# linhthi/BLISS-GNN

Measured on AMD Instinct MI355X. Metric: steps/sec (train step: sample_blocks + gather + SAGE fwd/bwd + Adam + exp3), reddit-like, higher is better.
Workload: dtype bf16

## Files before the change

bliss_gnn_amd/_lib.py:

```python
import ctypes as C
import os

_HERE = os.path.dirname(os.path.abspath(__file__))
LIB_PATH = os.path.join(_HERE, "libbliss_gnn.so")

EINVAL = -1
MODE_BANDIT, MODE_LADIES, MODE_UNIFORM_NODES, MODE_PARTIALS = 0, 1, 4, 8

ERR_BITS = {
    1: "frontier larger than 2^31-1 edges",
    2: "candidate capacity exceeded / seed id out of range",
    4: "kept-node capacity exceeded",
    8: "block-edge capacity exceeded",
    16: "non-finite or negative weight reached an exact reduction",
    32: "exact sum left its fixed-point range",
    64: "seed capacity exceeded",
    128: "random stream ran short / generator made no progress",
    256: "a cross-stream flag never came (bliss_flag_wait timed out)",
}


class Graph(C.Structure):
    _fields_ = [("indptr", C.c_void_p), ("indices", C.c_void_p), ("eid", C.c_void_p),
                ("num_nodes", C.c_int32), ("num_edges", C.c_int64)]
# ... 67 lines not shown
                ("rows_bound", C.c_int32), ("rows_dev", C.c_void_p),
                ("dw", C.c_void_p), ("dw_stride", C.c_int64), ("db", C.c_void_p)]


class GatFused(C.Structure):
    _fields_ = [("indptr", C.c_void_p), ("src", C.c_void_p), ("n_dst", C.c_int32), ("n_dst_dev", C.c_void_p),
                ("feat", C.c_void_p), ("feat_stride", C.c_int64), ("attn", C.c_void_p), ("heads", C.c_int32), ("head_dim", C.c_int32),
                ("negative_slope", C.c_float), ("e", C.c_void_p), ("a", C.c_void_p), ("a_drop", C.c_void_p),
                ("rst", C.c_void_p), ("rst_stride", C.c_int64),
                ("drop_p", C.c_float), ("drop_seed", C.c_uint32), ("drop_ctr", C.c_void_p), ("drop_ctr_used", C.c_void_p),
                ("g", C.c_void_p), ("g_stride", C.c_int64), ("de", C.c_void_p), ("d_er", C.c_void_p), ("d_er_stride", C.c_int64),
                ("dattn_part", C.c_void_p),
                ("wg_row", C.c_void_p), ("n_wg_dev", C.c_void_p), ("cap_wg", C.c_int32), ("row_ws", C.c_void_p), ("seg_part", C.c_void_p),
                ("err", C.c_void_p)]


ADAM_MAX_TENSORS = 32


class AdamTensors(C.Structure):
    _fields_ = [("param", C.c_void_p * ADAM_MAX_TENSORS), ("grad", C.c_void_p * ADAM_MAX_TENSORS),
                ("exp_avg", C.c_void_p * ADAM_MAX_TENSORS), ("exp_avg_sq", C.c_void_p * ADAM_MAX_TENSORS),
                ("numel", C.c_int64 * ADAM_MAX_TENSORS), ("count", C.c_int32)]


class BlockOut(C.Structure):
    _fields_ = [("indptr", C.c_void_p), ("src", C.c_void_p), ("dst", C.c_void_p), ("pos", C.c_void_p),
                ("eid", C.c_void_p), ("edge_weights", C.c_void_p), ("q_ij", C.c_void_p), ("t_indptr", C.c_void_p),
                ("t_edge", C.c_void_p), ("t_scratch", C.c_void_p), ("cap_b", C.c_int32)]


_P, _I32, _I64, _F, _D = C.c_void_p, C.c_int32, C.c_int64, C.c_float, C.c_double

SIGNATURES = {
    "bliss_layer_counts_bytes": [],
    "bliss_frontier_prob": [C.POINTER(Graph), C.POINTER(NodeMaps), _P, _P, _I32, _P, _I32, C.c_int, _F, _F, _I64, C.POINTER(LayerWs), _P],
    "bliss_rng_stream_begin": [_P, _P, _P, _P, _I32, _P],
    "bliss_rng_stream_wait": [_P, _P, _P, C.c_int, _I32, _P],
    "bliss_rng_stream_end": [_P, _P, _P, _I32, _P, _P],
    "bliss_rng_stream_chain": [_P, _P, _P, _P, _I32, _P, _I32, _P, _P],
    "bliss_rng_stream_ready": [_P],
    "bliss_rng_prepare": [_I32, _P],
    "bliss_mt_jump_poly": [_I64, _P],
    "bliss_flag_wait": [_P, _P, _P],
    "bliss_flag_set_spin_bound": [C.c_int64],
    "bliss_flag_raise": [_P, _P],
    "bliss_gather_rows": [_P, _I64, _P, _I32, _I32, _P, _I64, _P, _P],
    "bliss_exp3_apply_ranks": [C.POINTER(Exp3RankLists), _P, _P, _P, _P],
    "bliss_pack_lists": [C.POINTER(PackLists), _P, _P],
    "bliss_mt19937_uniform": [_P, _P, _I32, _P, _I32, _P],
    "bliss_poisson_select": [C.POINTER(LayerWs), _I32, _D, _P, _P, _P, C.c_int, _I32, _I64, _P],
    "bliss_multinomial_select": [C.POINTER(LayerWs), _P, _I32, _P],
    "bliss_tile_gemm": [C.POINTER(TileGemm), C.POINTER(TileGemm), _P],
    "bliss_cross_entropy": [_P, _I64, _P, _I32, _I32, _P, _P, _I64, _P, _P, _P, _P],
    "bliss_cross_entropy_sum": [_P, _I64, _P, _I64, _P, _P, _I32, _I32, _P, _P, _I64, _P, _P, _P, _P],
    "bliss_cross_entropy_masked": [_P, _I64, _P, _I64, _P, _I32, _P, _I32, _I32, _P, _F, _I32, _P, _P, _I64, _P, _P, _P, _P],
    "bliss_adam_step": [C.POINTER(AdamTensors), _P, _F, _F, _F, _F, _P],
    "bliss_cand_importance": [_P, _I32, C.c_int, _P, _P, _P],
    "bliss_poisson_scale": [_P, _P, _I32, _D, _P, _P],
    "bliss_keyed_select": [_P, _P, _P, _I32, _P, C.c_uint64, C.c_uint64, _I32, _P, _P, _P],
    "bliss_exp3_normalize_global": [_P, _I64, _P, _P, _P, _P, _P],
    "bliss_build_block": [C.POINTER(Graph), C.POINTER(NodeMaps), _P, _P, _I32, C.c_int, _F, _F, _I64, C.POINTER(LayerWs), C.POINTER(BlockOut), _P],
    "bliss_normalized_edata": [C.POINTER(Graph), _P, _P],
    "bliss_embed_norm": [_P, _I32, _I32, _I64, _P, _P],
    "bliss_spmm_fwd": [_P, _P, _P, _P, _P, _I64, _I32, _P, _I32, _I32, C.c_int, _P, _I64, C.c_int, _P, _P],
    "bliss_spmm_bwd": [_P, _P, _P, _P, _P, _P, _P, _I64, _I32, _P, _I32, _I32, C.c_int, _P, _I64, C.c_int, _P, _P],
    "bliss_block_transpose": [_P, _P, _I32, _I32, _I32, _P, _P, _P, _I64, _P],
    "bliss_spmm_chunk_edges": [_I32],
    "bliss_sage_epilogue_fwd": [_P, _I64, _P, _I64, _I32, _I32, _F, C.c_uint32, _P, _P, _I64, _P, _P],
    "bliss_sage_epilogue_bwd": [_P, _I64, _P, _I64, _I32, _I32, _F, _P, _I64, _P],
    "bliss_gat_chunk_edges": [],
    "bliss_graph_prepare": [_P, _P, _I64, _I32, C.c_int, _P, _P, _P, _P, _P, _P, _I64, _P],
    "bliss_exp3_update": [C.POINTER(Graph), _P, _P, _P, _P, _P, _P, _P, _P, _P, _P, _P, _P, _I32, _P, _I32, _F, _P, _P, C.c_int, _P, _P],
    "bliss_exp3_step": [C.POINTER(Graph), _P, C.POINTER(Exp3Block), _I32, _F, _P, _P],
    "bliss_exp3_normalize_global_rows": [C.POINTER(Exp3Block), _I32, _I64, _P, _I64, _P],
    "bliss_exp3_update_blocks": [C.POINTER(Graph), _P, C.POINTER(Exp3Block), _I32, _F, _P, _P],
    "bliss_exp3_apply": [_P, _P, _P, _P, _P, _I32, _P, _P],
    "bliss_exp3_normalize": [_P, _I64, _P, _P, _P, _P],
    "bliss_row_sum": [_P, _I64, _P, _P],
    "bliss_gat_logits": [_P, _P, _P, _I32, _P, _I64, _P, _I32, _I32, _F, _P, _P],
    "bliss_sage_dgrad": [C.POINTER(DGrad), _P],
    "bliss_sage_wgrad": [C.POINTER(WGrad), _I32, _P, _I64, _P],
    "bliss_shard_local_seeds": [_P, _I32, _P, _I32, _I32, _I32, _P, _P, _P, _P, _P, _P],
    "bliss_shard_scatter_partials": [_P, _P, _P, _P, _P, _P, _P, _I32, _P, _P],
    "bliss_shard_zero_dense": [_P, _I32, _P],
    "bliss_shard_pack_rows": [_P, _P, _I32, _I32, _I32, _P, _I64, _I32, _P, _I64, _P],
    "bliss_shard_place_rows": [_P, _I64, _P, _P, _I32, _P, _I64, _I32, _I32, _P],
    "bliss_shard_take_rows": [_P, _I32, _I64, _I32, _P, _P, _I32, _P, _I64, _I32, _P],
    "bliss_shard_candidates": [_P, _I32, _I32, _P, _P, _P, _P, _P, _I32, _P, _P, _P],
    "bliss_shard_select_kept": [_P, _P, _P, _P, C.c_uint64, _P, _I32, _P, _I32, _P, _P, _P, _P, _P, _I32, _I32, _I32, _P, _P, _P, _I32, _P, _P, _P],
    "bliss_gat_fused_supported": [_I32, _I32],
    "bliss_gat_segment_edges": [],
    "bliss_gat_fused_stamps": [_P, _P],
    "bliss_gat_segments": [_P, _I32, _I32, _P, _P, _P, _P],
    "bliss_gat_fused_fwd": [C.POINTER(GatFused), _P],
    "bliss_gat_fused_bwd_dst": [C.POINTER(GatFused), _P, _P, _P, _P],
    "bliss_gat_rows_src_fused": [_P, _I32, _P, _P, _P, _P, _I32, _P, _P, _P, _I64, _P, _I64, _P, _I32, _I32, _F, _P, _I64, _P, _P],
    "bliss_gat_logits_f32": [_P, _P, _P, _I32, _P, _I64, _P, _I32, _I32, _F, _P, _P],
    "bliss_gat_edge_dot": [_P, _P, _P, _I32, _P, _I64, _P, _I64, _I32, _I32, _P, _P],
    "bliss_gat_edge_softmax": [_P, _I32, _P, _P, _I32, C.c_int, _P, _P],
    "bliss_gat_rows": [C.c_int, _P, _I32, _P, _P, _P, _P, _I32, _P, _P, _I64, _P, _I32, _I32, _F, _P, _I64, _P, _P, _P],
    "bliss_gat_alpha": [_P, _I32, _P, _P, _P, _P, _P],
    "bliss_prof_enable": [C.c_int],
    "bliss_prof_reset": [],
    "bliss_prof_read": [C.c_int, C.POINTER(C.c_double), C.POINTER(C.c_int64)],
    "bliss_prof_kernel_count": [],
# ... 43 lines not shown
```

bliss_gnn_amd/csrc/sage.hip:

```cpp
#include "common.cuh"
#include "bliss_gnn.h"
#include <cstdlib>

namespace {

typedef __bf16 bf16x8_t __attribute__((ext_vector_type(8)));
typedef float f32x16_t __attribute__((ext_vector_type(16)));

#define TG_TPB 512
#define TG_M 32
#define TG_WAVES (TG_TPB / 64)
#define TG_NB (256 / 32 / TG_WAVES)

struct TileGemm {
  const bf16_t* a1; long long a1_stride; const int* ids;
  const bf16_t* w1; long long w1_stride; int k1;
  const bf16_t* a2; long long a2_stride; const bf16_t* w2; long long w2_stride; int k2;
  const bf16_t* bias;
  int m_bound; const int* m_dev; int n;
  bf16_t* out; long long out_stride;
  bf16_t* a_copy; long long copy_stride;
  bf16_t* in_norm; bf16_t* out_norm;
  int relu; unsigned drop_thresh; float drop_scale; unsigned seed; unsigned long long* ctr;
};
// ... 4 lines not shown
}

__device__ __forceinline__ uint32_t tg_drop_hash(uint32_t seed, uint32_t ctr, uint32_t idx) {
  uint32_t x = idx * 0x9e3779b1u + seed;
  x ^= ctr * 0x85ebca77u + 0x165667b1u;
  x ^= x >> 16; x *= 0x7feb352du; x ^= x >> 15; x *= 0x846ca68bu; x ^= x >> 16;
  x += ctr; x ^= x >> 15; x *= 0x2c1b3c6du; x ^= x >> 12;
  return x;
}

__device__ __forceinline__ float row_sumsq(const bf16_t* sh, int dim, int vec4, int lane) {
  float s = 0.f;
  if (vec4) {
    for (int c = lane * 4; c < dim; c += 256) {
      const float a = bf2f(sh[c]), b = bf2f(sh[c + 1]), cc = bf2f(sh[c + 2]), d = bf2f(sh[c + 3]);
      s += a * a; s += b * b; s += cc * cc; s += d * d;
    }
  } else {
    for (int c = lane; c < dim; c += 64) { const float a = bf2f(sh[c]); s += a * a; }
  }
  for (int d = 32; d >= 1; d >>= 1) s += __shfl_xor(s, d);
  return s;
}

__device__ __forceinline__ void rows_norm(const bf16_t* tile, int stride, int dim, int row0, int M, int m_bound, bf16_t* __restrict__ out,
                                          int wave, int lane) {
  constexpr int RPW = TG_M / TG_WAVES;
  float s[RPW];
#pragma unroll
  for (int q = 0; q < RPW; ++q) s[q] = 0.f;
  if (dim % 4 == 0) {
    for (int c = lane * 4; c < dim; c += 256)
#pragma unroll
      for (int q = 0; q < RPW; ++q) {
        const bf16_t* sh = tile + (size_t)(q * TG_WAVES + wave) * stride + c;
        const float a = bf2f(sh[0]), b = bf2f(sh[1]), cc = bf2f(sh[2]), d = bf2f(sh[3]);
        s[q] += a * a; s[q] += b * b; s[q] += cc * cc; s[q] += d * d;
      }
  } else {
    for (int c = lane; c < dim; c += 64)
#pragma unroll
      for (int q = 0; q < RPW; ++q) { const float a = bf2f(tile[(size_t)(q * TG_WAVES + wave) * stride + c]); s[q] += a * a; }
  }
  for (int d = 32; d >= 1; d >>= 1)
#pragma unroll
    for (int q = 0; q < RPW; ++q) s[q] += __shfl_xor(s[q], d);
#pragma unroll
  for (int q = 0; q < RPW; ++q) {
    const int r = row0 + q * TG_WAVES + wave;
    if (lane == 0 && r < m_bound) out[r] = r < M ? f2bf(sqrtf(s[q])) : (bf16_t)0;
  }
}

__device__ __forceinline__ void stage_rows(const bf16_t* __restrict__ a, long long a_stride, const int* row_id, int k,
                                           int row0, int m_bound, bf16_t* tile, int stride, bf16_t* __restrict__ copy, long long copy_stride,
                                           int wave, int lane) {
  const int kp = k_pad16(k);
  const bool even = (k % 2 == 0) && (a_stride % 2 == 0) && (((uintptr_t)a) % 4 == 0);
  const bool copy32 = copy && (copy_stride % 2 == 0) && (((uintptr_t)copy) % 4 == 0);
  if (even) {
    const int dw = k / 2;
    constexpr int MAXC = (1024 / 2 + 63) / 64;
    constexpr int RPW = TG_M / TG_WAVES, HALF = RPW;
#pragma unroll
    for (int hb = 0; hb < 1; ++hb) {
      uint32_t v[HALF][MAXC];
#pragma unroll
      for (int q = 0; q < HALF; ++q) {
        const int id = row_id[(hb * HALF + q) * TG_WAVES + wave];
        const uint32_t* src = reinterpret_cast<const uint32_t*>(a + (long long)(id < 0 ? 0 : id) * a_stride);
#pragma unroll
        for (int j = 0; j < MAXC; ++j) {
          const int c = lane + 64 * j;
          const uint32_t x = src[c < dw ? c : dw - 1];
          v[q][j] = (id >= 0 && c < dw) ? x : 0u;
        }
      }
#pragma unroll
      for (int q = 0; q < HALF; ++q) {
        const int lr = (hb * HALF + q) * TG_WAVES + wave, r = row0 + lr;
        uint32_t* sh = reinterpret_cast<uint32_t*>(tile + (size_t)lr * stride);
#pragma unroll
        for (int j = 0; j < MAXC; ++j) {
          const int c = lane + 64 * j;
          if (c < kp / 2) sh[c] = v[q][j];
          if (copy && r < m_bound && c < dw) {
            if (copy32) reinterpret_cast<uint32_t*>(copy + (long long)r * copy_stride)[c] = v[q][j];
            else { bf16_t* cp = copy + (long long)r * copy_stride + 2 * c; cp[0] = (bf16_t)(v[q][j] & 0xffffu); cp[1] = (bf16_t)(v[q][j] >> 16); }
          }
        }
      }
    }
  } else {
    for (int rd = 0; rd < TG_M / TG_WAVES; ++rd) {
      const int lr = rd * TG_WAVES + wave, r = row0 + lr, id = row_id[lr];
      const bf16_t* src = a + (long long)(id < 0 ? 0 : id) * a_stride;
      bf16_t* sh = tile + (size_t)lr * stride;
      for (int c = lane; c < kp; c += 64) {
        const bf16_t x = (id >= 0 && c < k) ? src[c] : (bf16_t)0;
        sh[c] = x;
        if (copy && r < m_bound && c < k) copy[(long long)r * copy_stride + c] = x;
      }
    }
  }
}

#define TG_SLAB 64
#define TG_WSTRIDE (TG_SLAB + 8)
#define TG_WROWS 256
typedef uint32_t u32x4_a4 __attribute__((ext_vector_type(4), aligned(4)));

struct WRegs { uint4 v[TG_WROWS * TG_SLAB / 8 / TG_TPB]; };

__device__ __forceinline__ void w_slab_load_full(WRegs& g, const bf16_t* __restrict__ w, long long w_stride, int N, int slab, int tid) {
  const int part = tid & 7, k = slab * TG_SLAB + 8 * part;
#pragma unroll
  for (int i = 0; i < (int)(sizeof(g.v) / sizeof(g.v[0])); ++i) {
    int n = i * (TG_TPB / 8) + (tid >> 3);
    n = n < N ? n : N - 1;
    const u32x4_a4 q = *reinterpret_cast<const u32x4_a4*>(w + (long long)n * w_stride + k);
    g.v[i] = make_uint4(q[0], q[1], q[2], q[3]);
  }
}
__device__ __forceinline__ void w_slab_load_tail(WRegs& g, const bf16_t* __restrict__ w, long long w_stride, int N, int K, int slab, int tid) {
  const int part = tid & 7, k = slab * TG_SLAB + 8 * part;
  for (int i = 0; i < (int)(sizeof(g.v) / sizeof(g.v[0])); ++i) {
    int n = i * (TG_TPB / 8) + (tid >> 3);
    n = n < N ? n : N - 1;
    const bf16_t* p = w + (long long)n * w_stride + k;
    union { uint4 u; bf16_t e[8]; } t;
    t.u = make_uint4(0, 0, 0, 0);
    for (int j = 0; j < 8; ++j) if (k + j < K) t.e[j] = p[j];
    g.v[i] = t.u;
  }
}
__device__ __forceinline__ int w_full_slabs(const bf16_t* w, long long w_stride, int K) {
  return ((w_stride % 2 == 0) && (((uintptr_t)w) % 4 == 0)) ? K / TG_SLAB : 0;
}
__device__ __forceinline__ void w_slab_store(const WRegs& g, bf16_t* wl, int tid) {
  const int part = tid & 7;
#pragma unroll
  for (int i = 0; i < (int)(sizeof(g.v) / sizeof(g.v[0])); ++i) {
    const int n = i * (TG_TPB / 8) + (tid >> 3);
    *reinterpret_cast<uint4*>(wl + (size_t)n * TG_WSTRIDE + 8 * part) = g.v[i];
  }
}

__device__ __forceinline__ void mma_product(WRegs& ga, WRegs& gb, const bf16_t* tile, int stride, int k, const bf16_t* __restrict__ w,
                                            long long w_stride, int n0, int N, bf16_t* wl, int tid, int lane, f32x16_t acc[TG_NB]) {
  const int kp = k_pad16(k), r = lane & 31, h = lane >> 5;
  const int nslab = (kp + TG_SLAB - 1) / TG_SLAB;
  auto multiply = [&](int sl) {
    if (n0 < N) {
#pragma unroll
      for (int st = 0; st < TG_SLAB / 16; ++st) {
        const int ks = sl * TG_SLAB + 16 * st;
        if (ks < kp) {
          const bf16x8_t a = *reinterpret_cast<const bf16x8_t*>(tile + (size_t)r * stride + ks + 8 * h);
#pragma unroll
          for (int nb = 0; nb < TG_NB; ++nb) {
            const bf16x8_t b = *reinterpret_cast<const bf16x8_t*>(wl + (size_t)(n0 + 32 * nb + r) * TG_WSTRIDE + 16 * st + 8 * h);
            acc[nb] = __builtin_amdgcn_mfma_f32_32x32x16_bf16(a, b, acc[nb], 0, 0, 0);
          }
        }
      }
    }
  };
  const int nfull = w_full_slabs(w, w_stride, k);
  for (int sl = 0; sl < nfull; sl += 2) {
    __syncthreads();
    w_slab_store(ga, wl, tid);
    if (sl + 2 < nfull) w_slab_load_full(ga, w, w_stride, N, sl + 2, tid);
    __syncthreads();
    multiply(sl);
    if (sl + 1 < nfull) {
      __syncthreads();
      w_slab_store(gb, wl, tid);
      if (sl + 3 < nfull) w_slab_load_full(gb, w, w_stride, N, sl + 3, tid);
      __syncthreads();
      multiply(sl + 1);
    }
  }
  for (int sl = nfull; sl < nslab; ++sl) {
    WRegs t;
    w_slab_load_tail(t, w, w_stride, N, k, sl, tid);
    __syncthreads();
    w_slab_store(t, wl, tid);
    __syncthreads();
    multiply(sl);
  }
}

__device__ __forceinline__ void tile_gemm_body(const TileGemm& p, bf16_t* lds, int* row_id, int dbg) {
  const int tid = threadIdx.x, wave = tid >> 6, lane = tid & 63;
  int M = p.m_bound;
  if (p.m_dev) { const int t = *p.m_dev; M = t < M ? t : M; }
  const int row0 = blockIdx.x * TG_M;
  const uint32_t ctr = p.drop_thresh ? (uint32_t)__hip_atomic_load(p.ctr, __ATOMIC_RELAXED, __HIP_MEMORY_SCOPE_AGENT) : 0u;
  const int N = p.n;
  if (row0 >= p.m_bound) return;
  if (row0 >= M) {
    for (int lr = wave; lr < TG_M; lr += TG_WAVES) {
      const int r = row0 + lr;
      if (r >= p.m_bound) break;
      for (int c = lane; c < N; c += 64) p.out[(long long)r * p.out_stride + c] = 0;
      if (p.a_copy) for (int c = lane; c < p.k1; c += 64) p.a_copy[(long long)r * p.copy_stride + c] = 0;
      if (lane == 0) { if (p.in_norm) p.in_norm[r] = 0; if (p.out_norm) p.out_norm[r] = 0; }
    }
    return;
  }
  const int s1 = lds_stride(p.k1), s2 = p.k2 ? lds_stride(p.k2) : 0;
  bf16_t* t1 = lds;
  bf16_t* t2 = lds + (size_t)TG_M * s1;
  const int n0 = wave * 32 * TG_NB;
  bf16_t* wl = lds + (size_t)TG_M * (s1 + s2);
  float bias_v[TG_NB];
#pragma unroll
  for (int nb = 0; nb < TG_NB; ++nb) bias_v[nb] = 0.f;
#pragma unroll
  for (int nb = 0; nb < TG_NB; ++nb) { const int col = n0 + 32 * nb + (lane & 31); if (p.bias && col < N) bias_v[nb] = bf2f(p.bias[col]); }
  WRegs ga, gb;
  {
    const int nf = w_full_slabs(p.w1, p.w1_stride, p.k1);
    if (nf > 0) w_slab_load_full(ga, p.w1, p.w1_stride, N, 0, tid);
    if (nf > 1) w_slab_load_full(gb, p.w1, p.w1_stride, N, 1, tid);
  }
  if (tid < TG_M) {
    const int r = row0 + tid;
    row_id[tid] = r < M ? (p.ids ? p.ids[r] : r) : -1;
    row_id[TG_M + tid] = r < M ? r : -1;
  }
  __syncthreads();
  if (!(dbg & 1)) stage_rows(p.a1, p.a1_stride, row_id, p.k1, row0, p.m_bound, t1, s1, p.a_copy, p.copy_stride, wave, lane);
  if (p.k2) stage_rows(p.a2, p.a2_stride, row_id + TG_M, p.k2, row0, p.m_bound, t2, s2, nullptr, 0, wave, lane);
  __syncthreads();
  if (p.in_norm && !(dbg & 4)) rows_norm(t1, s1, p.k1, row0, M, p.m_bound, p.in_norm, wave, lane);
  f32x16_t acc[TG_NB];
#pragma unroll
  for (int m = 0; m < TG_NB; ++m)
#pragma unroll
    for (int i = 0; i < 16; ++i) acc[m][i] = 0.f;
  if (!(dbg & 2)) mma_product(ga, gb, t1, s1, p.k1, p.w1, p.w1_stride, n0, N, wl, tid, lane, acc);
  if (p.k2) {
    const int nf = w_full_slabs(p.w2, p.w2_stride, p.k2);
    if (nf > 0) w_slab_load_full(ga, p.w2, p.w2_stride, N, 0, tid);
    if (nf > 1) w_slab_load_full(gb, p.w2, p.w2_stride, N, 1, tid);
    mma_product(ga, gb, t2, s2, p.k2, p.w2, p.w2_stride, n0, N, wl, tid, lane, acc);
  }
  __syncthreads();
  const int so = ((N + 63) & ~63) + 8;
  bf16_t* ot = lds;
  if (n0 < N) {
#pragma unroll
    for (int m = 0; m < TG_NB; ++m) {
      const int col = n0 + 32 * m + (lane & 31);
      const float bv = bias_v[m];
#pragma unroll
      for (int i = 0; i < 16; ++i) {
        const int lr = (i & 3) + 8 * (i >> 2) + 4 * (lane >> 5);
        float t = rbf(acc[m][i] + bv);
        if (p.relu) t = t > 0.f ? t : 0.f;
        if (p.drop_thresh) {
          const bool keep = tg_drop_hash(p.seed, ctr, (uint32_t)((row0 + lr) * N + col)) >= p.drop_thresh;
          t = keep ? rbf(t * p.drop_scale) : 0.f;
        }
        ot[(size_t)lr * so + col] = (row0 + lr < M && col < N) ? f2bf(t) : (bf16_t)0;
      }
    }
  }
  __syncthreads();
  const bool pair_ok = (N % 2 == 0) && (p.out_stride % 2 == 0) && (((uintptr_t)p.out) % 4 == 0);
  for (int lr = wave; lr < TG_M; lr += TG_WAVES) {
    const int r = row0 + lr;
    if (r >= p.m_bound) break;
    const bf16_t* sh = ot + (size_t)lr * so;
    bf16_t* o = p.out + (long long)r * p.out_stride;
    if (pair_ok) for (int c = lane * 2; c < N; c += 128) *reinterpret_cast<uint32_t*>(o + c) = *reinterpret_cast<const uint32_t*>(sh + c);
    else for (int c = lane; c < N; c += 64) o[c] = sh[c];
  }
  if (p.out_norm) rows_norm(ot, so, N, row0, M, p.m_bound, p.out_norm, wave, lane);
}

__global__ void __launch_bounds__(TG_TPB) k_tile_gemm(TileGemm p0, TileGemm p1, int n_sets, int dbg) {
  extern __shared__ __attribute__((aligned(16))) bf16_t tg_lds[];
  __shared__ int row_id[2 * TG_M];
  if (dbg & 8) return;
  tile_gemm_body(blockIdx.y == 0 ? p0 : p1, tg_lds, row_id, dbg);
  unsigned long long* ctr = p0.drop_thresh ? p0.ctr : (n_sets > 1 && p1.drop_thresh ? p1.ctr : nullptr);
  if (ctr) {
    __syncthreads();
    if (threadIdx.x == 0) {
      const unsigned long long total = (unsigned long long)gridDim.x * gridDim.y;
      if (atomicAdd(ctr + 1, 1ull) == total - 1) {
        __hip_atomic_store(ctr + 1, 0ull, __ATOMIC_RELAXED, __HIP_MEMORY_SCOPE_AGENT);
        atomicAdd(ctr, 1ull);
      }
    }
  }
}

bool convert(const bliss_tile_gemm_t* a, TileGemm* p, size_t* lds_bytes, int* tiles) {
  if (!a->a1 || !a->w1 || !a->out || a->k1 <= 0 || a->k1 > 1024 || a->n <= 0 || a->n > 256 || a->m_bound <= 0) return false;
  if (a->k2 < 0 || a->k2 > 1024 || (a->k2 > 0 && (!a->a2 || !a->w2))) return false;
  if (a->drop_p < 0.f || a->drop_p >= 1.f || (a->drop_p > 0.f && !a->drop_ctr)) return false;
  p->a1 = (const bf16_t*)a->a1; p->a1_stride = a->a1_stride; p->ids = a->ids;
  p->w1 = (const bf16_t*)a->w1; p->w1_stride = a->w1_stride; p->k1 = a->k1;
  p->a2 = (const bf16_t*)a->a2; p->a2_stride = a->a2_stride; p->w2 = (const bf16_t*)a->w2; p->w2_stride = a->w2_stride; p->k2 = a->k2;
  p->bias = (const bf16_t*)a->bias; p->m_bound = a->m_bound; p->m_dev = a->m_dev; p->n = a->n;
  p->out = (bf16_t*)a->out; p->out_stride = a->out_stride; p->a_copy = (bf16_t*)a->a_copy; p->copy_stride = a->copy_stride;
  p->in_norm = (bf16_t*)a->in_norm; p->out_norm = (bf16_t*)a->out_norm; p->relu = a->relu;
  p->drop_thresh = a->drop_p > 0.f ? (unsigned)((double)a->drop_p * 4294967296.0) : 0u;
  p->drop_scale = a->drop_p > 0.f ? 1.0f / (1.0f - a->drop_p) : 1.0f;
  p->seed = a->drop_seed; p->ctr = (unsigned long long*)a->drop_ctr;
  const size_t stage = ((size_t)TG_M * (lds_stride(a->k1) + (a->k2 ? lds_stride(a->k2) : 0)) + (size_t)TG_WROWS * TG_WSTRIDE) * sizeof(bf16_t);
  const size_t outt = (size_t)TG_M * (((a->n + 63) & ~63) + 8) * sizeof(bf16_t);
  *lds_bytes = stage > outt ? stage : outt;
  *tiles = (a->m_bound + TG_M - 1) / TG_M;
  return true;
}

}

extern "C" int bliss_tile_gemm(const bliss_tile_gemm_t* first, const bliss_tile_gemm_t* second, void* stream) {
  if (!first) return BLISS_EINVAL;
  TileGemm p0, p1;
  size_t l0 = 0, l1 = 0;
  int t0 = 0, t1 = 0;
  if (!convert(first, &p0, &l0, &t0)) return BLISS_EINVAL;
  p1 = p0;
  if (second && !convert(second, &p1, &l1, &t1)) return BLISS_EINVAL;
  const size_t lds = l0 > l1 ? l0 : l1;
  if (lds > 160 * 1024) return BLISS_EINVAL;
  static size_t lds_set = 0;
  if (lds > lds_set) {
    if (hipFuncSetAttribute((const void*)k_tile_gemm, hipFuncAttributeMaxDynamicSharedMemorySize, (int)lds) != hipSuccess) return BLISS_EINVAL;
    lds_set = lds;
  }
  const dim3 grid(t0 > t1 ? t0 : t1, second ? 2 : 1);
  static const int dbg = []() { const char* e = getenv("BLISS_TG_DEBUG"); return e ? atoi(e) : 0; }();
  k_tile_gemm<<<grid, TG_TPB, lds, (hipStream_t)stream>>>(p0, p1, second ? 2 : 1, dbg);
  return (int)hipGetLastError();
}
```

include/bliss_gnn.h:

```cpp
#ifndef BLISS_GNN_H
#define BLISS_GNN_H
#include <stdint.h>

#ifdef __cplusplus
extern "C" {
#endif

#define BLISS_EINVAL (-1)

#define BLISS_MODE_BANDIT 0
#define BLISS_MODE_LADIES 1
#define BLISS_ROWSUM_SLOTS 32
#define BLISS_NORM_SCRATCH (2 + 3 * BLISS_ROWSUM_SLOTS)
#define BLISS_MODE_UNIFORM_NODES 4
#define BLISS_MODE_PARTIALS 8

typedef struct {
  const int64_t* indptr;
  const int32_t* indices;
  const int32_t* eid;
  int32_t num_nodes;
  int64_t num_edges;
} bliss_graph_t;

// ... 79 lines not shown
                      int64_t frontier_bound, const bliss_layer_ws_t* ws, const bliss_block_out_t* out, void* stream);

int bliss_mt19937_uniform(void* state, const int32_t* n_dev, int32_t n_word_offset, float* out, int32_t cap, void* stream);

int bliss_rng_stream_begin(const void* state, int32_t* ctl, float* out, uint32_t* raw, int32_t cap_total, void* stream);
int bliss_rng_prepare(int32_t cap_total, int32_t* plan4);
int bliss_mt_jump_poly(int64_t n_words, uint32_t* poly_words);
int bliss_rng_stream_wait(int32_t* ctl, const void* counts, int32_t* layer_off, int is_last, int32_t cap_total, void* stream);
int bliss_rng_stream_end(void* state, const int32_t* ctl, const uint32_t* raw, int32_t cap_total, int32_t* err_word,
                         void* stream);
int bliss_rng_stream_chain(void* state, int32_t* ctl, float* out, uint32_t* raw, int32_t cap_total, int32_t* counts_dev,
                           int32_t n_count_words, int32_t* counts_host, void* stream);
int bliss_rng_stream_ready(void* stream);
int64_t bliss_rng_stream_handle(void);

int bliss_cand_importance(const int64_t* sums, int32_t n, int uniform_nodes, void* p_bf16, int32_t* err, void* stream);
int bliss_poisson_scale(int32_t* hist, void* counts, int32_t fanout, double eps, int32_t* scratch, void* stream);
int bliss_keyed_select(const int32_t* nid, const void* p_bf16, const uint8_t* is_seed, int32_t n, const void* counts,
                       uint64_t seed, uint64_t step, int32_t layer, void* P_bf16, uint8_t* keep, void* stream);
int bliss_shard_local_seeds(const int32_t* seeds_g, int32_t n_seeds, const int32_t* n_seeds_dev, int32_t lo, int32_t hi, int32_t cap_s,
                            int32_t* seeds_l, int32_t* seeds_l_copy, int32_t* seed_pos, int32_t* n_local_dev, int32_t* err, void* stream);
int bliss_shard_scatter_partials(const int32_t* seeds_l, const int64_t* seed_p2, const int32_t* n_local_dev, const int64_t* touched_key,
                                 const int64_t* touched_sum, const int32_t* n_touched_dev, int64_t* dense, int32_t num_nodes,
                                 int32_t* err, void* stream);
int bliss_shard_pack_rows(const int32_t* nid, const int32_t* n_rows_dev, int32_t cap_rows, int32_t lo, int32_t hi, const void* table_bf16,
                          int64_t table_stride, int32_t row_len, void* out_bf16, int64_t out_stride, void* stream);
int bliss_shard_place_rows(const void* src_bf16, int64_t src_stride, const int32_t* pos, const int32_t* n_dev, int32_t cap_s, void* out_bf16,
                           int64_t out_stride, int32_t n_rows, int32_t row_len, void* stream);
int bliss_shard_take_rows(const void* src, int32_t src_is_f32, int64_t src_stride, int32_t n_src_rows, const int32_t* pos, const int32_t* n_dev,
                          int32_t cap_s, void* out_bf16, int64_t out_stride, int32_t row_len, void* stream);
int bliss_shard_zero_dense(int64_t* dense, int32_t num_nodes, void* stream);
int bliss_shard_candidates(int64_t* dense, int32_t num_nodes, int32_t uniform_nodes, int32_t* cand_nid, void* p_bf16, uint8_t* is_seed,
                           int32_t* hist, void* counts, int32_t cap_c, int32_t* scratch, int32_t* err, void* stream);
int bliss_shard_select_kept(const int32_t* cand_nid, const void* p_bf16, const uint8_t* is_seed, const void* counts, uint64_t seed,
                            int64_t* step_dev, int32_t layer, const int32_t* seeds_g, int32_t n_seeds, const int32_t* n_seeds_dev,
                            void* P_bf16, int32_t* kept_nid, void* node_prob_bf16, int32_t* kept_map, int32_t cap_k, int32_t cap_c,
                            int32_t num_nodes, void* layer_counts, const int32_t* n_local_dev, int32_t* scratch, int32_t bump_step,
                            int32_t* done_flag, int32_t* err, void* stream);
int bliss_exp3_normalize_global(void* w_pos, int64_t num_edges, int64_t* row_sum, const int64_t* norm_limbs, int64_t* scratch,
                                void* norm_out_bf16, void* stream);

typedef struct {
  const void* a1; int64_t a1_stride; const int32_t* ids;
  const void* w1; int64_t w1_stride; int32_t k1;
  const void* a2; int64_t a2_stride; const void* w2; int64_t w2_stride; int32_t k2;
  const void* bias;
  int32_t m_bound; const int32_t* m_dev; int32_t n;
  void* out; int64_t out_stride;
  void* a_copy; int64_t copy_stride;
  void* in_norm; void* out_norm;
  int32_t relu; float drop_p; uint32_t drop_seed; void* drop_ctr;
} bliss_tile_gemm_t;
int bliss_tile_gemm(const bliss_tile_gemm_t* first, const bliss_tile_gemm_t* second_or_null, void* stream);

typedef struct {
  const void* a1; int64_t a1_stride; const void* w1; int64_t w1_stride; int32_t k1;
  const void* a2; int64_t a2_stride; const void* w2; int64_t w2_stride; int32_t k2; int32_t m2_bound; const int32_t* m2_dev;
  int32_t m_bound; const int32_t* m_dev; int32_t n;
  void* out; int64_t out_stride;
} bliss_dgrad_t;
int bliss_sage_dgrad(const bliss_dgrad_t* args, void* stream);
typedef struct {
  const void* d; int64_t d_stride; int32_t n_out;
  const void* x; int64_t x_stride; int32_t k_in;
  int32_t rows_bound; const int32_t* rows_dev;
  void* dw; int64_t dw_stride; void* db;
} bliss_wgrad_t;
int64_t bliss_sage_wgrad_workspace(const bliss_wgrad_t* probs, int32_t n_probs);
int bliss_sage_wgrad(const bliss_wgrad_t* probs, int32_t n_probs, float* partials, int64_t partial_floats, void* stream);

int bliss_cross_entropy(const void* logits, int64_t stride, const int64_t* labels, int32_t n_rows, int32_t n_cls,
                        float* row_loss, void* dlogits, int64_t d_stride, float* loss_out, uint32_t* ticket, int32_t* err,
                        void* stream);
int bliss_cross_entropy_sum(const void* logits, int64_t stride, const void* logits2, int64_t stride2, const int64_t* label_table,
                            const int32_t* label_ids, int32_t n_rows, int32_t n_cls, float* row_loss, void* dlogits, int64_t d_stride,
                            float* loss_out, uint32_t* ticket, int32_t* err, void* stream);
int bliss_cross_entropy_masked(const void* logits, int64_t stride, const void* logits2, int64_t stride2, const int64_t* label_table,
                               int32_t n_table, const int32_t* label_ids, int32_t id_off, int32_t n_rows, const int32_t* n_rows_dev,
                               float denom, int32_t n_cls, float* row_loss, void* dlogits, int64_t d_stride, float* loss_out,
                               uint32_t* ticket, int32_t* err, void* stream);

#define BLISS_ADAM_MAX_TENSORS 32
typedef struct {
  void* param[BLISS_ADAM_MAX_TENSORS];
  const void* grad[BLISS_ADAM_MAX_TENSORS];
  void* exp_avg[BLISS_ADAM_MAX_TENSORS];
  void* exp_avg_sq[BLISS_ADAM_MAX_TENSORS];
  int64_t numel[BLISS_ADAM_MAX_TENSORS];
  int32_t count;
} bliss_adam_t;
int bliss_adam_step(const bliss_adam_t* tensors, float* state, float beta1, float beta2, float eps, float weight_decay, void* stream);

int bliss_normalized_edata(const bliss_graph_t* g, void* w_pos, void* stream);

int bliss_gather_rows(const void* feat, int64_t feat_stride, const int32_t* ids, int32_t n_rows, int32_t dim, void* out,
                      int64_t out_stride, void* norm_out, void* stream);

int bliss_embed_norm(const void* h, int32_t n_rows, int32_t dim, int64_t row_stride, void* out, void* stream);

int bliss_spmm_chunk_edges(int32_t nnz_bound);
int bliss_spmm_fwd(const int32_t* indptr, const int32_t* src, const int32_t* dst, const void* w, const void* h,
                   int64_t h_stride, int32_t n_dst, const int32_t* nnz_dev, int32_t nnz, int32_t dim, int mean, void* out,
                   int64_t out_stride, int out_fp32, float* partials, void* stream);

int bliss_spmm_bwd(const int32_t* t_indptr, const int32_t* t_edge, const int32_t* src, const int32_t* dst,
                   const int32_t* indptr, const void* w, const void* gout, int64_t gout_stride, int32_t n_src,
// ... 114 lines not shown
```

scratch/tgbench.py:

```python
import sys, os, torch
sys.path.insert(0, os.path.dirname(os.path.dirname(os.path.abspath(__file__))))
from bliss_gnn_amd import nn as bnn
dev = torch.device("cuda")
g = torch.Generator().manual_seed(0)
def timeit(fn, n=20):
    st = torch.cuda.Stream()
    with torch.cuda.stream(st):
        for _ in range(3): fn()
    torch.cuda.synchronize()
    gr = torch.cuda.CUDAGraph()
    with torch.cuda.graph(gr):
        for _ in range(n): fn()
    gr.replay(); torch.cuda.synchronize()
    a, b = torch.cuda.Event(enable_timing=True), torch.cuda.Event(enable_timing=True)
    a.record(); gr.replay(); gr.replay(); b.record(); torch.cuda.synchronize()
    return a.elapsed_time(b) / (2 * n) * 1e3
V, F = 232965, 602
table = torch.randn(V, F, generator=g).bfloat16().to(dev)
for name, K, S, Kin, N, gather in (("L0 pair (gather)", 11100, 4900, 602, 256, True), ("L0 pair exact", 7300, 3300, 602, 256, True),
                                   ("L2 pair", 1900, 256, 256, 41, False)):
    ids = torch.randint(0, V, (K,), generator=g).to(torch.int32).to(dev)
    x = table if gather else torch.randn(K, Kin, generator=g).bfloat16().to(dev)
    wn = torch.randn(N, Kin, generator=g).bfloat16().to(dev); ws = torch.randn(N, Kin, generator=g).bfloat16().to(dev); b = torch.randn(N).bfloat16().to(dev)
    z = torch.empty(K, N, dtype=torch.bfloat16, device=dev); y = torch.empty(S, N, dtype=torch.bfloat16, device=dev)
    rows = torch.empty(K, Kin, dtype=torch.bfloat16, device=dev); nrm = torch.empty(K, dtype=torch.bfloat16, device=dev)
    a1 = bnn._tg_args(x, wn, z, K, ids=ids if gather else None, a_copy=rows if gather else None, in_norm=nrm)
    a2 = bnn._tg_args(x, ws, y, S, ids=ids if gather else None, bias=b)
    t = timeit(lambda: bnn._tile_gemm(a1, a2))
    def lib():
        xx = table[ids.long()] if gather else x
        torch.nn.functional.linear(xx, wn); torch.nn.functional.linear(xx[:S], ws, b)
    print(f"{name:20s} tile_gemm {t:7.1f} us   library (gather + 2 linear) {timeit(lib):7.1f} us")
S, D = 1900, 256
agg = torch.randn(S, D, generator=g).bfloat16().to(dev); h = torch.randn(4900, D, generator=g).bfloat16().to(dev)
wn = torch.randn(D, D, generator=g).bfloat16().to(dev); ws = torch.randn(D, D, generator=g).bfloat16().to(dev); b = torch.randn(D).bfloat16().to(dev)
out = torch.empty(S, D, dtype=torch.bfloat16, device=dev); nrm = torch.empty(S, dtype=torch.bfloat16, device=dev)
a = bnn._tg_args(agg, wn, out, S, a2=h[:S], w2=ws, bias=b, out_norm=nrm, relu=True)
print(f"{'L1 dual':20s} tile_gemm {timeit(lambda: bnn._tile_gemm(a)):7.1f} us   library {timeit(lambda: torch.relu(torch.nn.functional.linear(agg, wn) + torch.nn.functional.linear(h[:S], ws, b))):7.1f} us")
```

Before: 1463.

## Pipeline tile GEMM weight slabs with unaligned-K loads and batched row staging

Adds a PIPE variant of the tile GEMM kernel, on by default. It loads weight slabs for any even K, including the K tail such as 602, by clamping the offset and shifting inside registers, so the tail no longer takes a serial unpipelined path. Both activation row sets are loaded into registers before either is written to LDS, which overlaps the gather latency of the two operands, and the weight prefetch is issued after the row-id setup. It also adds wall-clock stamp instrumentation behind a device pointer for per-phase profiling, at the cost of larger register use and extra branch code.

```diff
diff --git a/bliss_gnn_amd/_lib.py b/bliss_gnn_amd/_lib.py
--- a/bliss_gnn_amd/_lib.py
+++ b/bliss_gnn_amd/_lib.py
@@ -143,6 +143,7 @@
     "bliss_poisson_select": [C.POINTER(LayerWs), _I32, _D, _P, _P, _P, C.c_int, _I32, _I64, _P],
     "bliss_multinomial_select": [C.POINTER(LayerWs), _P, _I32, _P],
     "bliss_tile_gemm": [C.POINTER(TileGemm), C.POINTER(TileGemm), _P],
+    "bliss_tile_gemm_stamps": [_P],
     "bliss_cross_entropy": [_P, _I64, _P, _I32, _I32, _P, _P, _I64, _P, _P, _P, _P],
     "bliss_cross_entropy_sum": [_P, _I64, _P, _I64, _P, _P, _I32, _I32, _P, _P, _I64, _P, _P, _P, _P],
     "bliss_cross_entropy_masked": [_P, _I64, _P, _I64, _P, _I32, _P, _I32, _I32, _P, _F, _I32, _P, _P, _I64, _P, _P, _P, _P],
diff --git a/bliss_gnn_amd/csrc/sage.hip b/bliss_gnn_amd/csrc/sage.hip
--- a/bliss_gnn_amd/csrc/sage.hip
+++ b/bliss_gnn_amd/csrc/sage.hip
@@ -80,6 +80,47 @@
   }
 }
 
+template <int MAXC> struct RowRegs { uint32_t v[TG_M / TG_WAVES][MAXC]; };
+__device__ __forceinline__ bool rows_even(const bf16_t* a, long long a_stride, int k) {
+  return (k % 2 == 0) && (a_stride % 2 == 0) && (((uintptr_t)a) % 4 == 0);
+}
+template <int MAXC>
+__device__ __forceinline__ void rows_load(RowRegs<MAXC>& g, const bf16_t* __restrict__ a, long long a_stride, const int* row_id, int k,
+                                          int wave, int lane) {
+  const int dw = k / 2;
+#pragma unroll
+  for (int q = 0; q < TG_M / TG_WAVES; ++q) {
+    const int id = row_id[q * TG_WAVES + wave];
+    const uint32_t* src = reinterpret_cast<const uint32_t*>(a + (long long)(id < 0 ? 0 : id) * a_stride);
+#pragma unroll
+    for (int j = 0; j < MAXC; ++j) {
+      const int c = lane + 64 * j;
+      const uint32_t x = src[c < dw ? c : dw - 1];
+      g.v[q][j] = (id >= 0 && c < dw) ? x : 0u;
+    }
+  }
+}
+template <int MAXC>
+__device__ __forceinline__ void rows_to_lds(const RowRegs<MAXC>& g, int k, int row0, int m_bound, bf16_t* tile, int stride,
+                                           bf16_t* __restrict__ copy, long long copy_stride, int wave, int lane) {
+  const int kp = k_pad16(k), dw = k / 2;
+  const bool copy32 = copy && (copy_stride % 2 == 0) && (((uintptr_t)copy) % 4 == 0);
+#pragma unroll
+  for (int q = 0; q < TG_M / TG_WAVES; ++q) {
+    const int lr = q * TG_WAVES + wave, r = row0 + lr;
+    uint32_t* sh = reinterpret_cast<uint32_t*>(tile + (size_t)lr * stride);
+#pragma unroll
+    for (int j = 0; j < MAXC; ++j) {
+      const int c = lane + 64 * j;
+      if (c < kp / 2) sh[c] = g.v[q][j];
+      if (copy && r < m_bound && c < dw) {
+        if (copy32) reinterpret_cast<uint32_t*>(copy + (long long)r * copy_stride)[c] = g.v[q][j];
+        else { bf16_t* cp = copy + (long long)r * copy_stride + 2 * c; cp[0] = (bf16_t)(g.v[q][j] & 0xffffu); cp[1] = (bf16_t)(g.v[q][j] >> 16); }
+      }
+    }
+  }
+}
+
 __device__ __forceinline__ void stage_rows(const bf16_t* __restrict__ a, long long a_stride, const int* row_id, int k,
                                            int row0, int m_bound, bf16_t* tile, int stride, bf16_t* __restrict__ copy, long long copy_stride,
                                            int wave, int lane) {
@@ -174,8 +215,61 @@
   }
 }
 
+__device__ __forceinline__ bool w_any_ok(const bf16_t* w, long long w_stride, int K) {
+  return (w_stride % 2 == 0) && (((uintptr_t)w) % 4 == 0) && K % 2 == 0 && K >= 8;
+}
+__device__ __forceinline__ void w_slab_load_any(WRegs& g, const bf16_t* __restrict__ w, long long w_stride, int N, int K, int slab,
+                                                int nslab, int tid) {
+  int live = slab < nslab;
+  asm volatile("" : "+v"(live));
+  const int part = tid & 7, k = slab * TG_SLAB + 8 * part;
+  const int kk = k + 8 <= K ? k : K - 8;
+#pragma unroll
+  for (int i = 0; i < (int)(sizeof(g.v) / sizeof(g.v[0])); ++i) {
+    int n = i * (TG_TPB / 8) + (tid >> 3);
+    n = n < N ? n : N - 1;
+    const long long off = ((long long)n * w_stride + kk) & -(long long)live;
+    const u32x4_a4 q = *reinterpret_cast<const u32x4_a4*>(w + off);
+    g.v[i] = make_uint4(q[0], q[1], q[2], q[3]);
+  }
+}
+__device__ __forceinline__ void w_slab_store_any(const WRegs& g, bf16_t* wl, int K, int slab, int tid) {
+  const int part = tid & 7, k = slab * TG_SLAB + 8 * part;
+  const int kk = k + 8 <= K ? k : K - 8, sh = (k - kk) / 2;
+  const uint32_t m0 = 0u - (uint32_t)(sh == 0), m1 = 0u - (uint32_t)(sh == 1), m2 = 0u - (uint32_t)(sh == 2), m3 = 0u - (uint32_t)(sh == 3);
+  uint32_t in[4];
+#pragma unroll
+  for (int e = 0; e < 4; ++e) in[e] = 0u - (uint32_t)(k + 2 * e < K);
+#pragma unroll
+  for (int i = 0; i < (int)(sizeof(g.v) / sizeof(g.v[0])); ++i) {
+    const int n = i * (TG_TPB / 8) + (tid >> 3);
+    const uint4 q = g.v[i];
+    const uint32_t d0 = (q.x & m0) | (q.y & m1) | (q.z & m2) | (q.w & m3), d1 = (q.y & m0) | (q.z & m1) | (q.w & m2),
+                   d2 = (q.z & m0) | (q.w & m1), d3 = q.w & m0;
+    *reinterpret_cast<uint4*>(wl + (size_t)n * TG_WSTRIDE + 8 * part) = make_uint4(d0 & in[0], d1 & in[1], d2 & in[2], d3 & in[3]);
+  }
+}
+
+template <bool ANY>
+__device__ __forceinline__ void w_prefetch(WRegs& ga, WRegs& gb, const bf16_t* __restrict__ w, long long w_stride, int N, int K, int tid) {
+  const int nf = ANY ? (k_pad16(K) + TG_SLAB - 1) / TG_SLAB : w_full_slabs(w, w_stride, K);
+  if (ANY) {
+    w_slab_load_any(ga, w, w_stride, N, K, 0, nf, tid);
+    w_slab_load_any(gb, w, w_stride, N, K, 1, nf, tid);
+  } else {
+    if (nf > 0) w_slab_load_full(ga, w, w_stride, N, 0, tid);
+    if (nf > 1) w_slab_load_full(gb, w, w_stride, N, 1, tid);
+  }
+}
+
+#define TG_NSTAMP 16
+__device__ long long* g_tg_stamps = nullptr;
+#define TG_STAMP(k) do { if (st && threadIdx.x == 0) st[(k)] = wall_clock64(); } while (0)
+
+template <bool ANY>
 __device__ __forceinline__ void mma_product(WRegs& ga, WRegs& gb, const bf16_t* tile, int stride, int k, const bf16_t* __restrict__ w,
-                                            long long w_stride, int n0, int N, bf16_t* wl, int tid, int lane, f32x16_t acc[TG_NB]) {
+                                            long long w_stride, int n0, int N, bf16_t* wl, int tid, int lane, f32x16_t acc[TG_NB],
+                                            long long* st, int s_full) {
   const int kp = k_pad16(k), r = lane & 31, h = lane >> 5;
   const int nslab = (kp + TG_SLAB - 1) / TG_SLAB;
   auto multiply = [&](int sl) {
@@ -194,6 +288,23 @@
       }
     }
   };
+  if (ANY) {
+    for (int sl = 0; sl < nslab; sl += 2) {
+      __syncthreads();
+      w_slab_store_any(ga, wl, k, sl, tid);
+      w_slab_load_any(ga, w, w_stride, N, k, sl + 2, nslab, tid);
+      __syncthreads();
+      multiply(sl);
+      __syncthreads();
+      w_slab_store_any(gb, wl, k, sl + 1, tid);
+      w_slab_load_any(gb, w, w_stride, N, k, sl + 3, nslab, tid);
+      __syncthreads();
+      multiply(sl + 1);
+    }
+    TG_STAMP(s_full);
+    TG_STAMP(s_full + 1);
+    return;
+  }
   const int nfull = w_full_slabs(w, w_stride, k);
   for (int sl = 0; sl < nfull; sl += 2) {
     __syncthreads();
@@ -209,6 +320,7 @@
       multiply(sl + 1);
     }
   }
+  TG_STAMP(s_full);
   for (int sl = nfull; sl < nslab; ++sl) {
     WRegs t;
     w_slab_load_tail(t, w, w_stride, N, k, sl, tid);
@@ -217,10 +329,23 @@
     __syncthreads();
     multiply(sl);
   }
-}
-
-__device__ __forceinline__ void tile_gemm_body(const TileGemm& p, bf16_t* lds, int* row_id, int dbg) {
+  TG_STAMP(s_full + 1);
+}
+
+template <int MAXC>
+__device__ __forceinline__ void stage_both(const TileGemm& p, const int* row_id, int row0, bf16_t* t1, int s1, bf16_t* t2, int s2,
+                                           int wave, int lane) {
+  RowRegs<MAXC> g1, g2;
+  rows_load<MAXC>(g1, p.a1, p.a1_stride, row_id, p.k1, wave, lane);
+  if (p.k2) rows_load<MAXC>(g2, p.a2, p.a2_stride, row_id + TG_M, p.k2, wave, lane);
+  rows_to_lds<MAXC>(g1, p.k1, row0, p.m_bound, t1, s1, p.a_copy, p.copy_stride, wave, lane);
+  if (p.k2) rows_to_lds<MAXC>(g2, p.k2, row0, p.m_bound, t2, s2, nullptr, 0, wave, lane);
+}
+
+template <bool PIPE>
+__device__ __forceinline__ void tile_gemm_body(const TileGemm& p, bf16_t* lds, int* row_id, int dbg, long long* st) {
   const int tid = threadIdx.x, wave = tid >> 6, lane = tid & 63;
+  TG_STAMP(0);
   int M = p.m_bound;
   if (p.m_dev) { const int t = *p.m_dev; M = t < M ? t : M; }
   const int row0 = blockIdx.x * TG_M;
@@ -235,6 +360,7 @@
       if (p.a_copy) for (int c = lane; c < p.k1; c += 64) p.a_copy[(long long)r * p.copy_stride + c] = 0;
       if (lane == 0) { if (p.in_norm) p.in_norm[r] = 0; if (p.out_norm) p.out_norm[r] = 0; }
     }
+    TG_STAMP(11);
     return;
   }
   const int s1 = lds_stride(p.k1), s2 = p.k2 ? lds_stride(p.k2) : 0;
@@ -248,34 +374,40 @@
 #pragma unroll
   for (int nb = 0; nb < TG_NB; ++nb) { const int col = n0 + 32 * nb + (lane & 31); if (p.bias && col < N) bias_v[nb] = bf2f(p.bias[col]); }
   WRegs ga, gb;
-  {
-    const int nf = w_full_slabs(p.w1, p.w1_stride, p.k1);
-    if (nf > 0) w_slab_load_full(ga, p.w1, p.w1_stride, N, 0, tid);
-    if (nf > 1) w_slab_load_full(gb, p.w1, p.w1_stride, N, 1, tid);
-  }
+  if (!PIPE) w_prefetch<false>(ga, gb, p.w1, p.w1_stride, N, p.k1, tid);
   if (tid < TG_M) {
     const int r = row0 + tid;
     row_id[tid] = r < M ? (p.ids ? p.ids[r] : r) : -1;
     row_id[TG_M + tid] = r < M ? r : -1;
   }
+  if (PIPE) w_prefetch<true>(ga, gb, p.w1, p.w1_stride, N, p.k1, tid);
   __syncthreads();
-  if (!(dbg & 1)) stage_rows(p.a1, p.a1_stride, row_id, p.k1, row0, p.m_bound, t1, s1, p.a_copy, p.copy_stride, wave, lane);
-  if (p.k2) stage_rows(p.a2, p.a2_stride, row_id + TG_M, p.k2, row0, p.m_bound, t2, s2, nullptr, 0, wave, lane);
+  TG_STAMP(1);
+  const bool even = rows_even(p.a1, p.a1_stride, p.k1) && (!p.k2 || rows_even(p.a2, p.a2_stride, p.k2));
+  const int kmax = p.k1 > p.k2 ? p.k1 : p.k2;
+  if (PIPE && even && !(dbg & 1) && kmax <= 256) stage_both<2>(p, row_id, row0, t1, s1, t2, s2, wave, lane);
+  else if (PIPE && even && !(dbg & 1) && kmax <= 512) stage_both<4>(p, row_id, row0, t1, s1, t2, s2, wave, lane);
+  else if (PIPE && even && !(dbg & 1) && kmax <= 640) stage_both<5>(p, row_id, row0, t1, s1, t2, s2, wave, lane);
+  else {
+    if (!(dbg & 1)) stage_rows(p.a1, p.a1_stride, row_id, p.k1, row0, p.m_bound, t1, s1, p.a_copy, p.copy_stride, wave, lane);
+    if (p.k2) stage_rows(p.a2, p.a2_stride, row_id + TG_M, p.k2, row0, p.m_bound, t2, s2, nullptr, 0, wave, lane);
+  }
   __syncthreads();
+  TG_STAMP(2);
   if (p.in_norm && !(dbg & 4)) rows_norm(t1, s1, p.k1, row0, M, p.m_bound, p.in_norm, wave, lane);
+  TG_STAMP(3);
   f32x16_t acc[TG_NB];
 #pragma unroll
   for (int m = 0; m < TG_NB; ++m)
 #pragma unroll
     for (int i = 0; i < 16; ++i) acc[m][i] = 0.f;
-  if (!(dbg & 2)) mma_product(ga, gb, t1, s1, p.k1, p.w1, p.w1_stride, n0, N, wl, tid, lane, acc);
+  if (!(dbg & 2)) mma_product<PIPE>(ga, gb, t1, s1, p.k1, p.w1, p.w1_stride, n0, N, wl, tid, lane, acc, st, 4);
   if (p.k2) {
-    const int nf = w_full_slabs(p.w2, p.w2_stride, p.k2);
-    if (nf > 0) w_slab_load_full(ga, p.w2, p.w2_stride, N, 0, tid);
-    if (nf > 1) w_slab_load_full(gb, p.w2, p.w2_stride, N, 1, tid);
-    mma_product(ga, gb, t2, s2, p.k2, p.w2, p.w2_stride, n0, N, wl, tid, lane, acc);
+    w_prefetch<PIPE>(ga, gb, p.w2, p.w2_stride, N, p.k2, tid);
+    mma_product<PIPE>(ga, gb, t2, s2, p.k2, p.w2, p.w2_stride, n0, N, wl, tid, lane, acc, st, 6);
   }
   __syncthreads();
+  TG_STAMP(8);
   const int so = ((N + 63) & ~63) + 8;
   bf16_t* ot = lds;
   if (n0 < N) {
@@ -297,6 +429,7 @@
     }
   }
   __syncthreads();
+  TG_STAMP(9);
   const bool pair_ok = (N % 2 == 0) && (p.out_stride % 2 == 0) && (((uintptr_t)p.out) % 4 == 0);
   for (int lr = wave; lr < TG_M; lr += TG_WAVES) {
     const int r = row0 + lr;
@@ -306,14 +439,21 @@
     if (pair_ok) for (int c = lane * 2; c < N; c += 128) *reinterpret_cast<uint32_t*>(o + c) = *reinterpret_cast<const uint32_t*>(sh + c);
     else for (int c = lane; c < N; c += 64) o[c] = sh[c];
   }
+  TG_STAMP(10);
   if (p.out_norm) rows_norm(ot, so, N, row0, M, p.m_bound, p.out_norm, wave, lane);
-}
-
+  TG_STAMP(11);
+}
+
+template <bool PIPE>
 __global__ void __launch_bounds__(TG_TPB) k_tile_gemm(TileGemm p0, TileGemm p1, int n_sets, int dbg) {
   extern __shared__ __attribute__((aligned(16))) bf16_t tg_lds[];
   __shared__ int row_id[2 * TG_M];
   if (dbg & 8) return;
-  tile_gemm_body(blockIdx.y == 0 ? p0 : p1, tg_lds, row_id, dbg);
+  long long* st = g_tg_stamps;
+  if (st) st += (long long)TG_NSTAMP * (blockIdx.y * gridDim.x + blockIdx.x);
+  const TileGemm& p = blockIdx.y == 0 ? p0 : p1;
+  if (PIPE && w_any_ok(p.w1, p.w1_stride, p.k1) && (!p.k2 || w_any_ok(p.w2, p.w2_stride, p.k2))) tile_gemm_body<true>(p, tg_lds, row_id, dbg, st);
+  else tile_gemm_body<false>(p, tg_lds, row_id, dbg, st);
   unsigned long long* ctr = p0.drop_thresh ? p0.ctr : (n_sets > 1 && p1.drop_thresh ? p1.ctr : nullptr);
   if (ctr) {
     __syncthreads();
@@ -349,6 +489,10 @@
 
 }
 
+extern "C" int bliss_tile_gemm_stamps(long long* stamps) {
+  return (int)hipMemcpyToSymbol(HIP_SYMBOL(g_tg_stamps), &stamps, sizeof(stamps));
+}
+
 extern "C" int bliss_tile_gemm(const bliss_tile_gemm_t* first, const bliss_tile_gemm_t* second, void* stream) {
   if (!first) return BLISS_EINVAL;
   TileGemm p0, p1;
@@ -359,13 +503,16 @@
   if (second && !convert(second, &p1, &l1, &t1)) return BLISS_EINVAL;
   const size_t lds = l0 > l1 ? l0 : l1;
   if (lds > 160 * 1024) return BLISS_EINVAL;
+  static const bool pipe = []() { const char* e = getenv("BLISS_TG_PIPE"); return !(e && e[0] == '0'); }();
+  const void* fn = pipe ? (const void*)k_tile_gemm<true> : (const void*)k_tile_gemm<false>;
   static size_t lds_set = 0;
   if (lds > lds_set) {
-    if (hipFuncSetAttribute((const void*)k_tile_gemm, hipFuncAttributeMaxDynamicSharedMemorySize, (int)lds) != hipSuccess) return BLISS_EINVAL;
+    if (hipFuncSetAttribute(fn, hipFuncAttributeMaxDynamicSharedMemorySize, (int)lds) != hipSuccess) return BLISS_EINVAL;
     lds_set = lds;
   }
   const dim3 grid(t0 > t1 ? t0 : t1, second ? 2 : 1);
   static const int dbg = []() { const char* e = getenv("BLISS_TG_DEBUG"); return e ? atoi(e) : 0; }();
-  k_tile_gemm<<<grid, TG_TPB, lds, (hipStream_t)stream>>>(p0, p1, second ? 2 : 1, dbg);
+  if (pipe) k_tile_gemm<true><<<grid, TG_TPB, lds, (hipStream_t)stream>>>(p0, p1, second ? 2 : 1, dbg);
+  else k_tile_gemm<false><<<grid, TG_TPB, lds, (hipStream_t)stream>>>(p0, p1, second ? 2 : 1, dbg);
   return (int)hipGetLastError();
 }
diff --git a/include/bliss_gnn.h b/include/bliss_gnn.h
--- a/include/bliss_gnn.h
+++ b/include/bliss_gnn.h
@@ -155,6 +155,7 @@
   int32_t relu; float drop_p; uint32_t drop_seed; void* drop_ctr;
 } bliss_tile_gemm_t;
 int bliss_tile_gemm(const bliss_tile_gemm_t* first, const bliss_tile_gemm_t* second_or_null, void* stream);
+int bliss_tile_gemm_stamps(long long* stamps);
 
 typedef struct {
   const void* a1; int64_t a1_stride; const void* w1; int64_t w1_stride; int32_t k1;
diff --git a/scratch/tgbench.py b/scratch/tgbench.py
--- a/scratch/tgbench.py
+++ b/scratch/tgbench.py
@@ -15,6 +15,24 @@
     a, b = torch.cuda.Event(enable_timing=True), torch.cuda.Event(enable_timing=True)
     a.record(); gr.replay(); gr.replay(); b.record(); torch.cuda.synchronize()
     return a.elapsed_time(b) / (2 * n) * 1e3
+from bliss_gnn_amd import _lib
+PHASES = [(0, 1, "ids"), (1, 2, "row gather"), (2, 3, "in-norms"), (3, 4, "W1 full slabs"), (4, 5, "W1 K tail"),
+          (5, 6, "W2 full slabs"), (6, 7, "W2 K tail"), (7, 8, "barrier"), (8, 9, "epilogue"), (9, 10, "store"), (10, 11, "out norms")]
+def stamps(fn, tiles):
+    buf = torch.zeros(tiles * 16, dtype=torch.int64, device=dev)
+    torch.cuda.synchronize()
+    _lib.check(_lib.lib.bliss_tile_gemm_stamps(buf.data_ptr()), "stamps")
+    fn(); torch.cuda.synchronize()
+    _lib.check(_lib.lib.bliss_tile_gemm_stamps(None), "stamps")
+    t = buf.view(tiles, 16).cpu().double()
+    t = t[(t[:, 11] > 0) & (t[:, 1] > 0)]
+    for a, b, _ in PHASES:
+        if b in (6, 7):
+            t[:, b] = torch.where(t[:, b] > 0, t[:, b], t[:, b - 1 if b == 7 else 5])
+    life = (t[:, 11] - t[:, 0]) / 100
+    print(f"    stamps: {t.shape[0]} workgroups, launch span {(t[:, 11].max() - t[:, 0].min()) / 100:.1f} us, "
+          f"start spread {(t[:, 0].max() - t[:, 0].min()) / 100:.1f} us, workgroup life mean {life.mean():.2f} max {life.max():.2f} us")
+    print("    " + "; ".join(f"{n} {((t[:, b] - t[:, a]) / 100).mean():.2f}" for a, b, n in PHASES))
 V, F = 232965, 602
 table = torch.randn(V, F, generator=g).bfloat16().to(dev)
 for name, K, S, Kin, N, gather in (("L0 pair (gather)", 11100, 4900, 602, 256, True), ("L0 pair exact", 7300, 3300, 602, 256, True),
@@ -27,6 +45,7 @@
     a1 = bnn._tg_args(x, wn, z, K, ids=ids if gather else None, a_copy=rows if gather else None, in_norm=nrm)
     a2 = bnn._tg_args(x, ws, y, S, ids=ids if gather else None, bias=b)
     t = timeit(lambda: bnn._tile_gemm(a1, a2))
+    stamps(lambda: bnn._tile_gemm(a1, a2), 2 * ((K + 31) // 32))
     def lib():
         xx = table[ids.long()] if gather else x
         torch.nn.functional.linear(xx, wn); torch.nn.functional.linear(xx[:S], ws, b)
@@ -37,3 +56,4 @@
 out = torch.empty(S, D, dtype=torch.bfloat16, device=dev); nrm = torch.empty(S, dtype=torch.bfloat16, device=dev)
 a = bnn._tg_args(agg, wn, out, S, a2=h[:S], w2=ws, bias=b, out_norm=nrm, relu=True)
 print(f"{'L1 dual':20s} tile_gemm {timeit(lambda: bnn._tile_gemm(a)):7.1f} us   library {timeit(lambda: torch.relu(torch.nn.functional.linear(agg, wn) + torch.nn.functional.linear(h[:S], ws, b))):7.1f} us")
+stamps(lambda: bnn._tile_gemm(a), (S + 31) // 32)
```

New measurement: 1476, median of 6. No clear change (+0.9%).
